# fircarpediem/LSS2_Multimodal_nu

Measured on AMD Instinct MI355X. Metric: BEV frames/sec (6-cam 352x128 -> 200x200x64), full hot path: CamEncode lift + splat + BevEncode, higher is better.
Workload: dtype bf16; 1 GPU; BASELINE configs[1]: model_BEV_TXT LSS hot path, batch=4/GPU, 6 cams 352x128, D=41, 200x200x64 BEV -> BevEncode -> 200x200x4, trunk (EfficientNet) not included: features are the input; batch_per_gpu=4, global_batch=4, parallelism=dp1 (sample-sharded, no collective), precision=bf16

## Files before the change

### lss2_multimodal_nu_amd/csrc/conv_ks.hip

```cpp
#include <stdlib.h>

#include <type_traits>

#include "lss_common.h"

namespace {

constexpr int KS_ROWS = 7;
constexpr int KS_POSB = 64;
constexpr int KS_LDS_MAX = 160 * 1024;

__device__ __attribute__((aligned(128))) unsigned char lss_ks_zero_page[128];

__device__ __forceinline__ void ks_glds16(const void* gsrc, void* lds_wave_base) {
  __builtin_amdgcn_global_load_lds((const __attribute__((address_space(1))) void*)gsrc,
                                   (__attribute__((address_space(3))) void*)lds_wave_base, 16, 0, 0);
}

template <int NCH, class Map>
__device__ __forceinline__ void ks_fill_patch(unsigned char* smem, const unsigned short* ximg, int Cin, int H, int W,
                                              int rows, int pitch, int nposp, int wave, int lane, Map map) {
  const int ppc = nposp >> 4;
  const int q64 = 64 / pitch, r64 = 64 - q64 * pitch;
  const int h = wave & 1;
  const int pos0 = 32 * (wave >> 1) + (lane >> 1);
  int pr = pos0 / pitch, pc = pos0 - pr * pitch;
  const unsigned char* zsrc = lss_ks_zero_page + (lane & 7) * 16;
  const unsigned short* xb = ximg + (2 * h + (lane & 1)) * 8;
  for (int i = wave; i < ppc; i += 4) {
    int iy, ix;
    map(pr, pc, iy, ix);
    const bool in = pr < rows && iy >= 0 && iy < H && ix >= 0 && ix < W;
    const unsigned short* src = xb + (in ? (iy * W + ix) * Cin : 0);
#pragma unroll
    for (int c = 0; c < NCH; ++c)
      ks_glds16(in ? (const void*)(src + c * 32) : (const void*)zsrc,
                smem + ((size_t)(c * 2 + h) * nposp + 32 * (i >> 1)) * 32);
    pr += q64; pc += r64;
    if (pc >= pitch) { pc -= pitch; ++pr; }
  }
}

struct KsStamps {
  unsigned long long* base;
  int tid;
  unsigned long long clk_main = 0;
  __device__ __forceinline__ void stamp(int k) const {
    if (base != nullptr && tid == 0) base[(size_t)blockIdx.x * 8 + k] = __builtin_amdgcn_s_memrealtime();
  }
  __device__ __forceinline__ void main_begin() {
    if (base != nullptr) clk_main = __builtin_amdgcn_s_memtime();
  }
  __device__ __forceinline__ void main_end(const f32x4& first, const f32x4& last) const {
    if (base != nullptr) asm volatile("s_nop 0" ::"v"(first), "v"(last));
    stamp(3);
    if (base != nullptr && tid == 0) base[(size_t)blockIdx.x * 8 + 7] = __builtin_amdgcn_s_memtime() - clk_main;
  }
  __device__ __forceinline__ void drain() const {
    if (base != nullptr) {
      stamp(5);
      asm volatile("s_waitcnt vmcnt(0)" ::: "memory");
      stamp(6);
    }
  }
};

__device__ __forceinline__ void ks_load_affine(const float* scale, const float* shift, int ch, float (&sc)[8], float (&sh)[8]) {
  f32x4 s0 = {1.f, 1.f, 1.f, 1.f}, s1 = s0, h0 = {0.f, 0.f, 0.f, 0.f}, h1 = h0;
  if (scale) { s0 = *reinterpret_cast<const f32x4*>(scale + ch); s1 = *reinterpret_cast<const f32x4*>(scale + ch + 4); }
  if (shift) { h0 = *reinterpret_cast<const f32x4*>(shift + ch); h1 = *reinterpret_cast<const f32x4*>(shift + ch + 4); }
#pragma unroll
  for (int i = 0; i < 4; ++i) { sc[i] = s0[i]; sc[4 + i] = s1[i]; sh[i] = h0[i]; sh[4 + i] = h1[i]; }
}

typedef __attribute__((ext_vector_type(4))) unsigned int u32x4;
__device__ __forceinline__ u32x4 ks_pack8(const float (&v)[8]) {
  return (u32x4){lss_pack_bf2(v[0], v[1]), lss_pack_bf2(v[2], v[3]), lss_pack_bf2(v[4], v[5]), lss_pack_bf2(v[6], v[7])};
}

__device__ __forceinline__ int ks_slot_tile(int slot, int kp, int pxt) {
  const int t = slot + kp;
  return t >= pxt ? t - pxt : t;
}

template <int PXT>
__device__ __forceinline__ void ks_slot_offsets(int (&ab)[PXT], int kp, int pl0, int x_first, int npx, int W,
                                                int rowpitch, int laneoff) {
  const int plast = npx - 1;
  const int yl = (x_first + plast) / W, xl = x_first + plast - yl * W;
  const int y0 = (x_first + pl0) / W, x0 = x_first + pl0 - y0 * W;
  int t = ks_slot_tile(0, kp, PXT);
  int pl = pl0 + t * 16;
  int y = (x_first + pl) / W, x = x_first + pl - y * W;
#pragma unroll
  for (int i = 0; i < PXT; ++i) {
    const bool live = pl < npx;
    ab[i] = ((live ? y : yl) * rowpitch + (live ? x : xl)) * 32 + laneoff;
    pl += 16; x += 16;
    if (x >= W) { x -= W; ++y; }
    if (++t == PXT) { t = 0; pl = pl0; x = x0; y = y0; }
  }
}

template <int NKW, int POS>
__device__ __forceinline__ f32x4 ks_sum_parts(const f32x4& own, const f32x4 (&g)[NKW - 1]) {
  f32x4 sum = POS == 0 ? own : g[0];
#pragma unroll
  for (int q = 1; q < NKW; ++q) {
    const f32x4 pv = q == POS ? own : g[q > POS ? q - 1 : q];
#pragma unroll
    for (int i = 0; i < 4; ++i) sum[i] += pv[i];
  }
  return sum;
}

template <int NKW>
__device__ __forceinline__ f32x4 ks_sum_lds(const f32x4* p0, int kstride) {
  f32x4 sum = p0[0];
#pragma unroll
  for (int k = 1; k < NKW; ++k) {
    const f32x4 pv = p0[k * kstride];
#pragma unroll
    for (int i = 0; i < 4; ++i) sum[i] += pv[i];
  }
  return sum;
}

template <int NKW, class F>
__device__ __forceinline__ void ks_for_pos(int kp, F&& f) {
  if constexpr (NKW == 2) f(std::integral_constant<int, 0>{});
  else if (kp < 2) f(std::integral_constant<int, 0>{});
  else if (kp == 2) f(std::integral_constant<int, 2>{});
  else f(std::integral_constant<int, 3>{});
}

template <bool RES>
__device__ __forceinline__ u32x4 ks_finish8(float (&v)[8], const float (&sc)[8], const float (&sh)[8], const uint4& rv,
                                            bool relu, bool split0) {
  const unsigned int ru[4] = {rv.x, rv.y, rv.z, rv.w};
#pragma unroll
  for (int i = 0; i < 8; ++i) {
    float r;
    if (split0 && i == 0) {
#pragma clang fp contract(off)
      const float p = v[i] * sc[i];
      r = p + sh[i];
    } else {
      r = __builtin_fmaf(v[i], sc[i], sh[i]);
    }
    if constexpr (RES) r += lss_bf2f((unsigned short)((i & 1) ? ru[i >> 1] >> 16 : ru[i >> 1] & 0xffff));
    v[i] = relu ? fmaxf(r, 0.f) : r;
  }
  return ks_pack8(v);
}

struct KsArgs {
  const unsigned short* x;
  const unsigned char* w;
  const float* scale;
  const float* shift;
  const unsigned short* residual;
  unsigned short* y;
  int B, H, W, Cin, Cout, relu, wt;
  int PB;
  int npb;
  int nposp;
  int ncb;
  unsigned long long* stamps;
};

template <int KSW, int NKW, int PXT>
__global__ __launch_bounds__(256, 1) void conv_ks_kernel(const KsArgs a) {
  static_assert(KSW % 9 == 0 && (NKW == 4 || NKW == 2), "a wave's K part is whole chunks of nine taps");
  static_assert(PXT >= NKW - 1, "ks_slot_tile: slot + kp < 2 PXT");
  constexpr int NPW = 4 / NKW;
  constexpr int CPW = KSW / 9;
  constexpr int NT = PXT * NPW;
  extern __shared__ __attribute__((aligned(1024))) unsigned char smem[];
  const int tid = threadIdx.x, lane = tid & 63;
  const int wave = __builtin_amdgcn_readfirstlane(tid >> 6);
  const int kp = wave % NKW, ph = wave / NKW;
  const int n = lane & 15, kq = lane >> 4;
  KsStamps st = {a.stamps, tid};
  st.stamp(0);

  const int t = lss_xcd_order(blockIdx.x, gridDim.x);
  const int cb = t % a.ncb;
  const int pbg = t / a.ncb;
  const int b = pbg / a.npb, pb = pbg - b * a.npb;
  const int HW = a.H * a.W, WP = a.W + 2;
  const int p0 = pb * a.PB;
  const int y_first = p0 / a.W;

  ks_fill_patch<NKW * KSW / 9>(smem, a.x + (size_t)b * HW * a.Cin, a.Cin, a.H, a.W, KS_ROWS, WP, a.nposp, wave, lane,
                               [&](int pr, int pc, int& iy, int& ix) { iy = y_first - 1 + pr; ix = pc - 1; });

#ifdef KS_WPRE_ALL
  constexpr int WPRE = KSW;
#else
  constexpr int WPRE = KSW >= 18 ? 8 : 5;
#endif
  bf16x8 wf[KSW][2];
  const unsigned char* wp = a.w + ((size_t)(cb * NKW + kp) * KSW * 2) * 1024 + lane * 16;
  auto load_w = [&](int s) {
#pragma unroll
    for (int ct = 0; ct < 2; ++ct) wf[s][ct] = *reinterpret_cast<const bf16x8*>(wp + (s * 2 + ct) * 1024);
  };
#pragma unroll
  for (int s = 0; s < WPRE; ++s) load_w(s);

  const int npx = min(a.PB, HW - p0);
  int ab[PXT];
  ks_slot_offsets<PXT>(ab, kp, ph * PXT * 16 + n, p0 - y_first * a.W, npx, a.W, WP,
                       (kq >> 1) * a.nposp * 32 + (kq & 1) * 16);
  st.stamp(1);
  constexpr int NOWN = (PXT + NKW - 1) / NKW;
  const int ch = cb * 32 + kq * 8;
  uint4 rres[NOWN];
#pragma unroll
  for (int k = 0; k < NOWN; ++k) {
    const int j = kp + k * NKW;
    const int pl = (ph * PXT + j) * 16 + n;
    rres[k] = make_uint4(0, 0, 0, 0);
    if (a.residual != nullptr && j < PXT && pl < npx)
      rres[k] = *reinterpret_cast<const uint4*>(a.residual + ((size_t)b * HW + p0 + pl) * a.Cout + ch);
  }
  float sc[8], sh[8];
  ks_load_affine(a.scale, a.shift, ch, sc, sh);
  f32x4 acc[PXT][2];
#pragma unroll
  for (int j = 0; j < PXT; ++j) {
    acc[j][0] = (f32x4){0.f, 0.f, 0.f, 0.f};
    acc[j][1] = (f32x4){0.f, 0.f, 0.f, 0.f};
  }
  asm volatile("s_waitcnt vmcnt(0)" ::: "memory");
  __syncthreads();
  st.stamp(2);

  bf16x8 fb[2][PXT];
  auto load_frags = [&](int buf, int s) {
    const unsigned char* cbase = smem + (size_t)(kp * CPW + s / 9) * a.nposp * KS_POSB;
    const int tap = s % 9;
    const int toff = ((tap / 3) * WP + (tap % 3)) * 32;
#pragma unroll
    for (int j = 0; j < PXT; ++j) fb[buf][j] = *reinterpret_cast<const bf16x8*>(cbase + ab[j] + toff);
  };
  st.main_begin();
  load_frags(0, 0);
#pragma unroll
  for (int s = 0; s < KSW; ++s) {
    if (s + WPRE < KSW) load_w(s + WPRE);
#ifndef KS_DIAG_NOREAD
    if (s + 1 < KSW) load_frags((s + 1) & 1, s + 1);
#endif
    __builtin_amdgcn_sched_barrier(0);
#pragma unroll
    for (int j = 0; j < PXT; ++j) {
#ifdef KS_DIAG_NOMFMA
      asm volatile("" :: "v"(fb[s & 1][j]), "v"(wf[s][0]), "v"(wf[s][1]));
#else
      acc[j][0] = __builtin_amdgcn_mfma_f32_16x16x32_bf16(wf[s][0], fb[s & 1][j], acc[j][0], 0, 0, 0);
      acc[j][1] = __builtin_amdgcn_mfma_f32_16x16x32_bf16(wf[s][1], fb[s & 1][j], acc[j][1], 0, 0, 0);
#endif
    }
    __builtin_amdgcn_sched_barrier(0);
  }

  st.main_end(acc[0][0], acc[PXT - 1][1]);
  __syncthreads();
  f32x4* part = reinterpret_cast<f32x4*>(smem);
#pragma unroll
  for (int i = 0; i < PXT; ++i) {
    if (i % NKW == 0 && kp + i < PXT) continue;
    const int tile = ph * PXT + ks_slot_tile(i, kp, PXT);
#pragma unroll
    for (int ct = 0; ct < 2; ++ct) part[((kp * NT + tile) * 2 + ct) * 64 + lane] = acc[i][ct];
  }
  __syncthreads();
  st.stamp(4);
  const __amdgpu_buffer_rsrc_t yrsrc = __builtin_amdgcn_make_buffer_rsrc(
      a.y, 0, a.wt ? (int)((size_t)a.B * HW * a.Cout * 2) : 0, 0x00020000);
  f32x4 fp[NOWN][2][NKW - 1];
#pragma unroll
  for (int k = 0; k < NOWN; ++k) {
    const int tile = ph * PXT + min(kp + k * NKW, PXT - 1);
#pragma unroll
    for (int ct = 0; ct < 2; ++ct)
#pragma unroll
      for (int m = 0; m < NKW - 1; ++m)
        fp[k][ct][m] = part[(((m < kp ? m : m + 1) * NT + tile) * 2 + ct) * 64 + lane];
  }
  __builtin_amdgcn_sched_barrier(0);
  f32x4 sum[NOWN][2];
  ks_for_pos<NKW>(kp, [&](auto pos) __attribute__((always_inline)) {
#pragma unroll
    for (int k = 0; k < NOWN; ++k)
#pragma unroll
      for (int ct = 0; ct < 2; ++ct) sum[k][ct] = ks_sum_parts<NKW, decltype(pos)::value>(acc[k * NKW][ct], fp[k][ct]);
  });
#pragma unroll
  for (int k = 0; k < NOWN; ++k) {
    const int j = kp + k * NKW;
    const int pl = (ph * PXT + j) * 16 + n;
    const bool live = j < PXT && pl < npx;
    const size_t o = ((size_t)b * HW + p0 + (live ? pl : 0)) * a.Cout + ch;
    float v[8];
#pragma unroll
    for (int ct = 0; ct < 2; ++ct)
#pragma unroll
      for (int i = 0; i < 4; ++i) v[4 * ct + i] = sum[k][ct][i];
    const u32x4 ov = ks_finish8<true>(v, sc, sh, rres[k], a.relu != 0, false);
    if (live) {
      if (a.wt) __builtin_amdgcn_raw_buffer_store_b128(ov, yrsrc, (int)(o * 2), 0, 16);
      else *reinterpret_cast<u32x4*>(a.y + o) = ov;
    }
  }
  st.drain();
}

__global__ void pack_weights_ks_kernel(const float* __restrict__ w, int Cout, int Cin, unsigned short* __restrict__ out,
                                       int dgrad) {
  const size_t ntot = (size_t)Cout * Cin * 9;
  for (size_t e = (size_t)blockIdx.x * 256 + threadIdx.x; e < ntot; e += (size_t)gridDim.x * 256) {
    const int j = e & 7;
    size_t r = e >> 3;
    const int l = r & 63; r >>= 6;
    const int ct = r & 1; r >>= 1;
    const int nks = (Cin >> 5) * 9;
    const int S = r % nks;
    const int cb = r / nks;
    const int m = l & 15, kq = l >> 4;
    const int co = cb * 32 + 8 * (m >> 2) + 4 * ct + (m & 3);
    const int ci = (S / 9) * 32 + kq * 8 + j;
    out[e] = lss_f2bf(dgrad ? w[((size_t)ci * Cout + co) * 9 + (8 - S % 9)] : w[((size_t)co * Cin + ci) * 9 + (S % 9)]);
  }
}

bool ks_enabled() {
  const char* e = getenv("LSS_CONV_KS");
  return e == nullptr || atoi(e) != 0;
}

unsigned long long* ks_stamps_from_env() {
  const char* e = getenv("LSS_KS_STAMPS");
  return e ? reinterpret_cast<unsigned long long*>(strtoull(e, nullptr, 16)) : nullptr;
}

int ks_pack_grid(size_t n) { return (int)((n + 255) / 256 > 4096 ? 4096 : (n + 255) / 256); }

template <class... P>
bool ks_aligned16(const P*... p) {
  return ((reinterpret_cast<uintptr_t>(p) | ...) & 15) == 0;
}

template <auto K, class Args>
int ks_launch(int grid, int lds, const Args& a, hipStream_t st) {
  static bool attr_set[64] = {};
  int dev = -1;
  if (hipGetDevice(&dev) != hipSuccess || dev < 0 || dev >= 64) dev = -1;
  if (dev < 0 || !attr_set[dev]) {
    hipError_t e = hipFuncSetAttribute(reinterpret_cast<const void*>(K), hipFuncAttributeMaxDynamicSharedMemorySize,
                                       KS_LDS_MAX);
    if (e != hipSuccess) return (int)e;
    if (dev >= 0) attr_set[dev] = true;
  }
  hipLaunchKernelGGL(K, dim3(grid), dim3(256), lds, st, a);
  return lss_launch_status();
}

struct KsPlan {
  int ok, lds, grid, variant;
  KsArgs a;
};

KsPlan ks_plan(int B, int H, int W, int Cin, int Cout) {
  KsPlan pl = {};
  KsArgs& p = pl.a;
  if (B <= 0 || H <= 0 || W < 4 || Cout <= 0 || Cout % 32 != 0) return pl;
  if (Cin == 256) { pl.variant = 0; p.PB = 80; }
  else if (Cin == 128) { pl.variant = 1; p.PB = 160; }
  else if (Cin == 64) { pl.variant = 2; p.PB = 320; }
  else return pl;
  p.B = B; p.H = H; p.W = W; p.Cin = Cin; p.Cout = Cout;
  const long long HW = (long long)H * W;
  if (p.PB > 4 * W + 1) return pl;
  p.npb = (int)((HW + p.PB - 1) / p.PB);
  p.ncb = Cout / 32;
  p.nposp = (KS_ROWS * (W + 2) + 31) / 32 * 32;
  const int patch = (Cin / 32) * p.nposp * KS_POSB;
  if (patch > 112 * 1024) return pl;
  const int ntile = p.PB / 16;
  const int red = (pl.variant == 2 ? 2 : 4) * ntile * 2 * 1024;
  pl.lds = patch > red ? patch : red;
  if (pl.lds > KS_LDS_MAX) return pl;
  const long long grid = (long long)B * p.npb * p.ncb;
  if (grid < 64 || grid > 512) return pl;
  if ((long long)B * HW * (Cin > Cout ? Cin : Cout) >= (1LL << 30)) return pl;
  pl.grid = (int)grid;
  pl.ok = 1;
  return pl;
}

struct KsS2Args {
  const unsigned short* x;
  const unsigned char* w;
  const float* scale;
  const float* shift;
  unsigned short* y;
  unsigned short* y2;
  int B, H, W, Cin, Cout, relu;
  int Ho, Wo, pitch;
  int PB, npb, nposp, ncb;
  unsigned long long* stamps;
};

constexpr int KS2_PXT = 3;
constexpr int KS2_CT = 4;

template <int NKW>
__global__ __launch_bounds__(256, 1) void conv_ks_s2_dual_kernel(const KsS2Args a) {
  static_assert(NKW == 4 || NKW == 2, "one 32-channel chunk of nine taps per K part");
  constexpr int NPW = 4 / NKW, PXT = KS2_PXT, CT = KS2_CT, NT = PXT * NPW, NCH = NKW;
  constexpr bool OWN = NKW == 2;
  extern __shared__ __attribute__((aligned(1024))) unsigned char smem[];
  const int tid = threadIdx.x, lane = tid & 63;
  const int wave = __builtin_amdgcn_readfirstlane(tid >> 6);
  const int kp = wave % NKW, ph = wave / NKW;
  const int n = lane & 15, kq = lane >> 4;
  KsStamps st = {a.stamps, tid};
  st.stamp(0);

  const int t = lss_xcd_order(blockIdx.x, gridDim.x);
  const int cb = t % a.ncb;
  const int pbg = t / a.ncb;
  const int b = pbg / a.npb, pb = pbg - b * a.npb;
  const int HWo = a.Ho * a.Wo, WP = a.pitch;
  const int p0 = pb * a.PB;
  const int r0 = p0 / a.Wo;

  ks_fill_patch<NCH>(smem, a.x + (size_t)b * a.H * a.W * a.Cin, a.Cin, a.H, a.W, KS_ROWS, WP, a.nposp, wave, lane,
                     [&](int pr, int pc, int& iy, int& ix) {
                       iy = 2 * r0 - 1 + pr; ix = pc < a.Wo ? 2 * pc : 2 * (pc - a.Wo) - 1;
                     });

  constexpr int WPRE = 4;
  bf16x8 wf[9][CT], wd[CT];
  const unsigned char* wp = a.w + ((size_t)(cb * NKW + kp) * 10 * CT) * 1024 + lane * 16;
  auto load_w = [&](int s) {
#pragma unroll
    for (int ct = 0; ct < CT; ++ct) wf[s][ct] = *reinterpret_cast<const bf16x8*>(wp + (s * CT + ct) * 1024);
  };
#pragma unroll
  for (int s = 0; s < WPRE; ++s) load_w(s);
#pragma unroll
  for (int ct = 0; ct < CT; ++ct) wd[ct] = *reinterpret_cast<const bf16x8*>(wp + (9 * CT + ct) * 1024);

  const int npx = min(a.PB, HWo - p0);
  const int rot = OWN ? kp : 0;
  int ab[PXT];
  ks_slot_offsets<PXT>(ab, rot, ph * PXT * 16 + n, p0 - r0 * a.Wo, npx, a.Wo, 2 * WP,
                       (kq >> 1) * a.nposp * 32 + (kq & 1) * 16);
  st.stamp(1);
  f32x4 acc[PXT][CT], acc2[PXT][CT];
#pragma unroll
  for (int j = 0; j < PXT; ++j)
#pragma unroll
    for (int ct = 0; ct < CT; ++ct) {
      acc[j][ct] = (f32x4){0.f, 0.f, 0.f, 0.f};
      acc2[j][ct] = (f32x4){0.f, 0.f, 0.f, 0.f};
    }
  asm volatile("s_waitcnt vmcnt(0)" ::: "memory");
  __syncthreads();
  st.stamp(2);

  bf16x8 fb[2][PXT];
  auto load_frags = [&](int buf, int s) {
    const unsigned char* cbase = smem + (size_t)kp * a.nposp * KS_POSB;
    const int ky = s / 3, kx = s % 3;
    const int toff = (ky * WP + (kx == 1 ? 0 : kx == 0 ? a.Wo : a.Wo + 1)) * 32;
#pragma unroll
    for (int j = 0; j < PXT; ++j) fb[buf][j] = *reinterpret_cast<const bf16x8*>(cbase + ab[j] + toff);
  };
  st.main_begin();
  load_frags(0, 0);
#pragma unroll
  for (int s = 0; s < 9; ++s) {
    if (s + WPRE < 9) load_w(s + WPRE);
    if (s + 1 < 9) load_frags((s + 1) & 1, s + 1);
    __builtin_amdgcn_sched_barrier(0);
#pragma unroll
    for (int j = 0; j < PXT; ++j)
#pragma unroll
      for (int ct = 0; ct < CT; ++ct)
        acc[j][ct] = __builtin_amdgcn_mfma_f32_16x16x32_bf16(wf[s][ct], fb[s & 1][j], acc[j][ct], 0, 0, 0);
    if (s == 4) {
#pragma unroll
      for (int j = 0; j < PXT; ++j)
#pragma unroll
        for (int ct = 0; ct < CT; ++ct)
          acc2[j][ct] = __builtin_amdgcn_mfma_f32_16x16x32_bf16(wd[ct], fb[0][j], acc2[j][ct], 0, 0, 0);
    }
    __builtin_amdgcn_sched_barrier(0);
  }

  st.main_end(acc[0][0], acc[PXT - 1][CT - 1]);
  __syncthreads();
  f32x4* part = reinterpret_cast<f32x4*>(smem);
#pragma unroll
  for (int i = 0; i < PXT; ++i) {
    if (OWN && i % NKW == 0 && kp + i < PXT) continue;
    const int tile = ph * PXT + ks_slot_tile(i, rot, PXT);
#pragma unroll
    for (int ct = 0; ct < CT; ++ct) {
      part[(((0 * NKW + kp) * NT + tile) * CT + ct) * 64 + lane] = acc[i][ct];
      part[(((1 * NKW + kp) * NT + tile) * CT + ct) * 64 + lane] = acc2[i][ct];
    }
  }
  float sc[2][2][8], sh[2][2][8];
#pragma unroll
  for (int o = 0; o < 2; ++o)
#pragma unroll
    for (int g = 0; g < 2; ++g)
      ks_load_affine(a.scale, a.shift, o * a.Cout + cb * 64 + g * 32 + kq * 8, sc[o][g], sh[o][g]);
  __syncthreads();
  st.stamp(4);
  constexpr int NOWN = (PXT + NKW - 1) / NKW;
  if constexpr (!OWN) {
#pragma unroll
    for (int k = 0; k < NOWN; ++k) {
      const int j = kp + k * NKW;
      if (j >= PXT) break;
      const int tile = ph * PXT + j;
      const int pl = tile * 16 + n;
      const bool live = pl < npx;
      const size_t opix = ((size_t)b * HWo + p0 + (live ? pl : 0)) * a.Cout + cb * 64 + kq * 8;
#pragma unroll
      for (int o = 0; o < 2; ++o)
#pragma unroll
        for (int g = 0; g < 2; ++g) {
          float v[8];
#pragma unroll
          for (int tt = 0; tt < 2; ++tt) {
            const f32x4 sum = ks_sum_lds<NKW>(part + ((o * NKW * NT + tile) * CT + 2 * g + tt) * 64 + lane, NT * CT * 64);
#pragma unroll
            for (int i = 0; i < 4; ++i) v[4 * tt + i] = sum[i];
          }
#pragma unroll
          for (int i = 0; i < 8; ++i) {
            v[i] = v[i] * sc[o][g][i] + sh[o][g][i];
            if (o == 0 && a.relu) v[i] = fmaxf(v[i], 0.f);
          }
          if (live) *reinterpret_cast<u32x4*>((o == 0 ? a.y : a.y2) + opix + g * 32) = ks_pack8(v);
        }
    }
    st.drain();
    return;
  }
  f32x4 fp[NOWN][2][CT][NKW - 1];
#pragma unroll
  for (int k = 0; k < NOWN; ++k) {
    const int tile = ph * PXT + min(kp + k * NKW, PXT - 1);
#pragma unroll
    for (int o = 0; o < 2; ++o)
#pragma unroll
      for (int ct = 0; ct < CT; ++ct)
#pragma unroll
        for (int m = 0; m < NKW - 1; ++m)
          fp[k][o][ct][m] = part[(((o * NKW + (m < kp ? m : m + 1)) * NT + tile) * CT + ct) * 64 + lane];
  }
  __builtin_amdgcn_sched_barrier(0);
  f32x4 sum[NOWN][2][CT];
  ks_for_pos<NKW>(kp, [&](auto pos) __attribute__((always_inline)) {
#pragma unroll
    for (int k = 0; k < NOWN; ++k)
#pragma unroll
      for (int ct = 0; ct < CT; ++ct) {
        sum[k][0][ct] = ks_sum_parts<NKW, decltype(pos)::value>(acc[k * NKW][ct], fp[k][0][ct]);
        sum[k][1][ct] = ks_sum_parts<NKW, decltype(pos)::value>(acc2[k * NKW][ct], fp[k][1][ct]);
      }
  });
#pragma unroll
  for (int k = 0; k < NOWN; ++k) {
    const int j = kp + k * NKW;
    const int pl = (ph * PXT + j) * 16 + n;
    const bool live = j < PXT && pl < npx;
    const size_t opix = ((size_t)b * HWo + p0 + (live ? pl : 0)) * a.Cout + cb * 64 + kq * 8;
#pragma unroll
    for (int o = 0; o < 2; ++o)
#pragma unroll
      for (int g = 0; g < 2; ++g) {
        float v[8];
#pragma unroll
        for (int tt = 0; tt < 2; ++tt)
#pragma unroll
          for (int i = 0; i < 4; ++i) v[4 * tt + i] = sum[k][o][2 * g + tt][i];
        const u32x4 ov = ks_finish8<false>(v, sc[o][g], sh[o][g], make_uint4(0, 0, 0, 0), o == 0 && a.relu, o == 0);
        if (live) *reinterpret_cast<u32x4*>((o == 0 ? a.y : a.y2) + opix + g * 32) = ov;
      }
  }
  st.drain();
}

__global__ void pack_weights_ks_s2_dual_kernel(const float* __restrict__ w1, const float* __restrict__ wd, int Cout,
                                               int Cin, unsigned short* __restrict__ out) {
  const size_t ntot = (size_t)Cout * Cin * 10;
  const int nch = Cin >> 5;
  for (size_t e = (size_t)blockIdx.x * 256 + threadIdx.x; e < ntot; e += (size_t)gridDim.x * 256) {
    const int j = e & 7;
    size_t r = e >> 3;
    const int l = r & 63; r >>= 6;
    const int ct = r & 3; r >>= 2;
    const int s = r % 10; r /= 10;
    const int kp = r % nch;
    const int cb = r / nch;
    const int m = l & 15, kq = l >> 4;
    const int co = cb * 64 + 32 * (ct >> 1) + 8 * (m >> 2) + 4 * (ct & 1) + (m & 3);
    const int ci = kp * 32 + kq * 8 + j;
    out[e] = lss_f2bf(s < 9 ? w1[((size_t)co * Cin + ci) * 9 + s] : wd[(size_t)co * Cin + ci]);
  }
}

struct KsS2Plan {
  int ok, lds, grid, nkw;
  KsS2Args a;
};

KsS2Plan ks_s2_plan(int B, int H, int W, int Cin, int Cout) {
  KsS2Plan pl = {};
  KsS2Args& p = pl.a;
  if (B <= 0 || H < 2 || W < 4 || Cout <= 0 || Cout % 64 != 0) return pl;
  if (Cin == 128) pl.nkw = 4;
  else if (Cin == 64) pl.nkw = 2;
  else return pl;
  p.B = B; p.H = H; p.W = W; p.Cin = Cin; p.Cout = Cout;
  p.Ho = (H - 1) / 2 + 1; p.Wo = (W - 1) / 2 + 1;
  p.pitch = 2 * p.Wo + 1;
  p.PB = 16 * KS2_PXT * (4 / pl.nkw);
  if (p.PB > 2 * p.Wo + 1) return pl;
  const long long HWo = (long long)p.Ho * p.Wo;
  p.npb = (int)((HWo + p.PB - 1) / p.PB);
  p.ncb = Cout / 64;
  p.nposp = (KS_ROWS * p.pitch + 31) / 32 * 32;
  const int patch = (Cin / 32) * p.nposp * KS_POSB;
  if (patch > 112 * 1024) return pl;
  const int red = 2 * pl.nkw * (p.PB / 16) * KS2_CT * 1024;
  pl.lds = patch > red ? patch : red;
  if (pl.lds > KS_LDS_MAX) return pl;
  const long long grid = (long long)B * p.npb * p.ncb;
  if (grid < 64 || grid > 512) return pl;
  if ((long long)B * H * W * Cin >= (1LL << 30) || (long long)B * HWo * Cout >= (1LL << 30)) return pl;
  pl.grid = (int)grid;
  pl.ok = 1;
  return pl;
}

constexpr int ST_TH = 12, ST_TW = 16;
constexpr int ST_PR = 2 * ST_TH + 5, ST_PW = 2 * ST_TW + 5;
constexpr int ST_NE = ST_TW + 3;
constexpr int ST_NPOSP = (ST_PR * ST_PW + 31) / 32 * 32;
constexpr int ST_LDS = 2 * ST_NPOSP * KS_POSB;
constexpr int ST_KS = 98;
constexpr int ST_WPRE = 8;
constexpr int ST_PXT = ST_TH / 2;

struct KsStemArgs {
  const unsigned short* x;
  const unsigned char* w;
  const float* scale;
  const float* shift;
  unsigned short* y;
  int B, H, W, Cout, relu;
  int Ho, Wo, nty, ntx, ncb;
  unsigned long long* stamps;
};

__global__ __launch_bounds__(256, 1) void conv_ks_stem_kernel(const KsStemArgs a) {
  constexpr int PXT = ST_PXT, Cin = 64;
  extern __shared__ __attribute__((aligned(1024))) unsigned char smem[];
  const int tid = threadIdx.x, lane = tid & 63;
  const int wave = __builtin_amdgcn_readfirstlane(tid >> 6);
  const int g = wave & 1, ph = wave >> 1;
  const int n = lane & 15, kq = lane >> 4;
  KsStamps st = {a.stamps, tid};
  st.stamp(0);

  const int t = lss_xcd_order(blockIdx.x, gridDim.x);
  const int cb = t % a.ncb;
  const int tg = t / a.ncb;
  const int npi = a.nty * a.ntx;
  const int b = tg / npi, ti = tg - b * npi;
  const int ty = ti / a.ntx, tx = ti - ty * a.ntx;
  const int oy0 = ty * ST_TH, ox0 = tx * ST_TW;
  const int iy0 = 2 * oy0 - 3, ix0 = 2 * ox0 - 3;

  ks_fill_patch<2>(smem, a.x + (size_t)b * a.H * a.W * Cin, Cin, a.H, a.W, ST_PR, ST_PW, ST_NPOSP, wave, lane,
                   [&](int pr, int pc, int& iy, int& ix) {
                     iy = iy0 + pr; ix = ix0 + (pc < ST_NE ? 2 * pc : 2 * (pc - ST_NE) + 1);
                   });

  bf16x8 wf[ST_KS][2];
  const unsigned char* wp = a.w + ((size_t)cb * ST_KS * 4 + 2 * g) * 1024 + lane * 16;
  auto load_w = [&](int s) {
#pragma unroll
    for (int ct = 0; ct < 2; ++ct) wf[s][ct] = *reinterpret_cast<const bf16x8*>(wp + (s * 4 + ct) * 1024);
  };
#pragma unroll
  for (int s = 0; s < ST_WPRE; ++s) load_w(s);

  const int ab0 = (2 * (ph * PXT) * ST_PW + n) * 32 + (kq >> 1) * ST_NPOSP * 32 + (kq & 1) * 16;
  st.stamp(1);
  f32x4 acc[PXT][2];
#pragma unroll
  for (int j = 0; j < PXT; ++j) {
    acc[j][0] = (f32x4){0.f, 0.f, 0.f, 0.f};
    acc[j][1] = (f32x4){0.f, 0.f, 0.f, 0.f};
  }
  const int ch = cb * 64 + g * 32 + kq * 8;
  float sc[8], sh[8];
  ks_load_affine(a.scale, a.shift, ch, sc, sh);
  asm volatile("s_waitcnt vmcnt(0)" ::: "memory");
  __syncthreads();
  st.stamp(2);

  bf16x8 fb[2][PXT];
  auto load_frags = [&](int buf, int s) {
    const int tap = s >> 1, ky = tap / 7, kx = tap % 7;
    const int toff = (ky * ST_PW + ((kx & 1) ? ST_NE + (kx >> 1) : (kx >> 1))) * 32;
    const unsigned char* cbase = smem + (size_t)(s & 1) * 2 * ST_NPOSP * 32 + ab0 + toff;
#pragma unroll
    for (int j = 0; j < PXT; ++j) fb[buf][j] = *reinterpret_cast<const bf16x8*>(cbase + j * (2 * ST_PW * 32));
  };
  st.main_begin();
  load_frags(0, 0);
#pragma unroll
  for (int s = 0; s < ST_KS; ++s) {
    if (s + ST_WPRE < ST_KS) load_w(s + ST_WPRE);
    if (s + 1 < ST_KS) load_frags((s + 1) & 1, s + 1);
    __builtin_amdgcn_sched_barrier(0);
#pragma unroll
    for (int j = 0; j < PXT; ++j) {
      acc[j][0] = __builtin_amdgcn_mfma_f32_16x16x32_bf16(wf[s][0], fb[s & 1][j], acc[j][0], 0, 0, 0);
      acc[j][1] = __builtin_amdgcn_mfma_f32_16x16x32_bf16(wf[s][1], fb[s & 1][j], acc[j][1], 0, 0, 0);
    }
    __builtin_amdgcn_sched_barrier(0);
  }
  st.main_end(acc[0][0], acc[PXT - 1][1]);
  st.stamp(4);

  const int ox = ox0 + n;
#pragma unroll
  for (int j = 0; j < PXT; ++j) {
    const int oy = oy0 + ph * PXT + j;
    float v[8];
#pragma unroll
    for (int i = 0; i < 4; ++i) { v[i] = acc[j][0][i]; v[4 + i] = acc[j][1][i]; }
#pragma unroll
    for (int i = 0; i < 8; ++i) {
      v[i] = v[i] * sc[i] + sh[i];
      if (a.relu) v[i] = fmaxf(v[i], 0.f);
    }
    if (oy < a.Ho && ox < a.Wo)
      *reinterpret_cast<u32x4*>(a.y + (((size_t)b * a.Ho + oy) * a.Wo + ox) * a.Cout + ch) = ks_pack8(v);
  }
  st.drain();
}

__global__ void pack_weights_ks_stem_kernel(const float* __restrict__ w, int Cout, unsigned short* __restrict__ out) {
  const size_t ntot = (size_t)Cout * 64 * 49;
  for (size_t e = (size_t)blockIdx.x * 256 + threadIdx.x; e < ntot; e += (size_t)gridDim.x * 256) {
    const int j = e & 7;
    size_t r = e >> 3;
    const int l = r & 63; r >>= 6;
    const int ct = r & 3; r >>= 2;
    const int S = r % ST_KS;
    const int cb = r / ST_KS;
    const int m = l & 15, kq = l >> 4;
    const int co = cb * 64 + 32 * (ct >> 1) + 8 * (m >> 2) + 4 * (ct & 1) + (m & 3);
    const int ci = (S & 1) * 32 + kq * 8 + j;
    out[e] = lss_f2bf(w[((size_t)co * 64 + ci) * 49 + (S >> 1)]);
  }
}

struct KsStemPlan {
  int ok, grid;
  KsStemArgs a;
};

KsStemPlan ks_stem_plan(int B, int H, int W, int Cin, int Cout) {
  KsStemPlan pl = {};
  KsStemArgs& p = pl.a;
  if (B <= 0 || H <= 0 || W <= 0 || Cin != 64 || Cout <= 0 || Cout % 64 != 0) return pl;
  p.B = B; p.H = H; p.W = W; p.Cout = Cout;
  p.Ho = (H - 1) / 2 + 1; p.Wo = (W - 1) / 2 + 1;
  if (p.Ho < ST_TH || p.Wo < ST_TW) return pl;
  p.nty = (p.Ho + ST_TH - 1) / ST_TH; p.ntx = (p.Wo + ST_TW - 1) / ST_TW;
  p.ncb = Cout / 64;
  const long long grid = (long long)B * p.nty * p.ntx * p.ncb;
  if (grid < 32 || grid > 256) return pl;
  if ((long long)B * H * W * Cin >= (1LL << 30) || (long long)B * p.Ho * p.Wo * Cout >= (1LL << 30)) return pl;
  pl.grid = (int)grid;
  pl.ok = 1;
  return pl;
}

}

extern "C" int lss_conv2d_ks_ok(int B, int H, int W, int Cin, int Cout) {
  return ks_enabled() && ks_plan(B, H, W, Cin, Cout).ok;
}

extern "C" size_t lss_conv2d_ks_packed_weight_bytes(int Cout, int Cin) {
  if (Cout <= 0 || Cout % 32 != 0 || (Cin != 64 && Cin != 128 && Cin != 256)) return 0;
  return (size_t)Cout * Cin * 9 * 2;
}

extern "C" int lss_conv2d_pack_weights_ks(const float* w_oihw, int Cout, int Cin, void* w_packed, void* stream) {
  LSS_CHECK_PTR(w_oihw); LSS_CHECK_PTR(w_packed);
  if (lss_conv2d_ks_packed_weight_bytes(Cout, Cin) == 0) return LSS_E_SHAPE;
  hipLaunchKernelGGL(pack_weights_ks_kernel, dim3(ks_pack_grid((size_t)Cout * Cin * 9)), dim3(256), 0, lss_stream(stream), w_oihw, Cout, Cin,
                     reinterpret_cast<unsigned short*>(w_packed), 0);
  return lss_launch_status();
}

extern "C" int lss_conv2d_pack_weights_ks_dgrad(const float* w_oihw, int Cout, int Cin, void* w_packed, void* stream) {
  LSS_CHECK_PTR(w_oihw); LSS_CHECK_PTR(w_packed);
  if (lss_conv2d_ks_packed_weight_bytes(Cin, Cout) == 0) return LSS_E_SHAPE;
  hipLaunchKernelGGL(pack_weights_ks_kernel, dim3(ks_pack_grid((size_t)Cout * Cin * 9)), dim3(256), 0, lss_stream(stream), w_oihw, Cin, Cout,
                     reinterpret_cast<unsigned short*>(w_packed), 1);
  return lss_launch_status();
}

int lss_conv_ks_launch(const void* x, const void* w_ks, const float* scale, const float* shift, const void* residual,
                       void* y, int B, int H, int W, int Cin, int Cout, int relu, int wt, hipStream_t st) {
  KsPlan p = ks_plan(B, H, W, Cin, Cout);
  if (!p.ok) return LSS_E_SHAPE;
  if (relu != 0 && relu != 1) return LSS_E_LAYOUT;
  if (!ks_aligned16(x, y, w_ks, residual)) return LSS_E_ALIGN;
  KsArgs& a = p.a;
  a.x = reinterpret_cast<const unsigned short*>(x);
  a.w = reinterpret_cast<const unsigned char*>(w_ks);
  a.scale = scale; a.shift = shift;
  a.residual = reinterpret_cast<const unsigned short*>(residual);
  a.y = reinterpret_cast<unsigned short*>(y);
  a.relu = relu; a.wt = wt;
  a.stamps = ks_stamps_from_env();
  if (p.variant == 0) return ks_launch<conv_ks_kernel<18, 4, 5>>(p.grid, p.lds, a, st);
  if (p.variant == 1) return ks_launch<conv_ks_kernel<9, 4, 10>>(p.grid, p.lds, a, st);
  return ks_launch<conv_ks_kernel<9, 2, 10>>(p.grid, p.lds, a, st);
}

extern "C" int lss_conv2d_ks_s2_dual_ok(int B, int H, int W, int Cin, int Cout) {
  return ks_enabled() && ks_s2_plan(B, H, W, Cin, Cout).ok;
}

extern "C" size_t lss_conv2d_ks_s2_dual_packed_weight_bytes(int Cout, int Cin) {
  if (Cout <= 0 || Cout % 64 != 0 || (Cin != 64 && Cin != 128)) return 0;
  return (size_t)Cout * Cin * 10 * 2;
}

extern "C" int lss_conv2d_pack_weights_ks_s2_dual(const float* w1_oihw, const float* wd_oi, int Cout, int Cin,
                                                  void* w_packed, void* stream) {
  LSS_CHECK_PTR(w1_oihw); LSS_CHECK_PTR(wd_oi); LSS_CHECK_PTR(w_packed);
  if (lss_conv2d_ks_s2_dual_packed_weight_bytes(Cout, Cin) == 0) return LSS_E_SHAPE;
  hipLaunchKernelGGL(pack_weights_ks_s2_dual_kernel, dim3(ks_pack_grid((size_t)Cout * Cin * 10)), dim3(256), 0, lss_stream(stream), w1_oihw, wd_oi, Cout,
                     Cin, reinterpret_cast<unsigned short*>(w_packed));
  return lss_launch_status();
}

extern "C" int lss_conv2d_ks_s2_dual_fwd(const void* x, const void* w_packed, const float* scale, const float* shift,
                                         void* y, void* y2, int B, int H, int W, int Cin, int Cout, int relu,
                                         void* stream) {
  LSS_CHECK_PTR(x); LSS_CHECK_PTR(w_packed); LSS_CHECK_PTR(y); LSS_CHECK_PTR(y2);
  KsS2Plan p = ks_s2_plan(B, H, W, Cin, Cout);
  if (!p.ok) return LSS_E_SHAPE;
  if (relu != 0 && relu != 1) return LSS_E_LAYOUT;
  if (!ks_aligned16(x, y, y2, w_packed, scale, shift)) return LSS_E_ALIGN;
  KsS2Args& a = p.a;
  a.x = reinterpret_cast<const unsigned short*>(x);
  a.w = reinterpret_cast<const unsigned char*>(w_packed);
  a.scale = scale; a.shift = shift;
  a.y = reinterpret_cast<unsigned short*>(y);
  a.y2 = reinterpret_cast<unsigned short*>(y2);
  a.relu = relu;
  a.stamps = ks_stamps_from_env();
  return p.nkw == 4 ? ks_launch<conv_ks_s2_dual_kernel<4>>(p.grid, p.lds, a, lss_stream(stream))
                    : ks_launch<conv_ks_s2_dual_kernel<2>>(p.grid, p.lds, a, lss_stream(stream));
}

extern "C" int lss_conv2d_ks_stem_ok(int B, int H, int W, int Cin, int Cout) {
  return ks_enabled() && ks_stem_plan(B, H, W, Cin, Cout).ok;
}

extern "C" size_t lss_conv2d_ks_stem_packed_weight_bytes(int Cout, int Cin) {
  if (Cout <= 0 || Cout % 64 != 0 || Cin != 64) return 0;
  return (size_t)Cout * Cin * 49 * 2;
}

extern "C" int lss_conv2d_pack_weights_ks_stem(const float* w_oihw, int Cout, int Cin, void* w_packed, void* stream) {
  LSS_CHECK_PTR(w_oihw); LSS_CHECK_PTR(w_packed);
  if (lss_conv2d_ks_stem_packed_weight_bytes(Cout, Cin) == 0) return LSS_E_SHAPE;
  hipLaunchKernelGGL(pack_weights_ks_stem_kernel, dim3(ks_pack_grid((size_t)Cout * Cin * 49)), dim3(256), 0, lss_stream(stream), w_oihw, Cout,
                     reinterpret_cast<unsigned short*>(w_packed));
  return lss_launch_status();
}

extern "C" int lss_conv2d_ks_stem_fwd(const void* x, const void* w_packed, const float* scale, const float* shift,
                                      void* y, int B, int H, int W, int Cin, int Cout, int relu, void* stream) {
  LSS_CHECK_PTR(x); LSS_CHECK_PTR(w_packed); LSS_CHECK_PTR(y);
  KsStemPlan p = ks_stem_plan(B, H, W, Cin, Cout);
  if (!p.ok) return LSS_E_SHAPE;
  if (relu != 0 && relu != 1) return LSS_E_LAYOUT;
  if (!ks_aligned16(x, y, w_packed, scale, shift)) return LSS_E_ALIGN;
  KsStemArgs& a = p.a;
  a.x = reinterpret_cast<const unsigned short*>(x);
  a.w = reinterpret_cast<const unsigned char*>(w_packed);
  a.scale = scale; a.shift = shift;
  a.y = reinterpret_cast<unsigned short*>(y);
  a.relu = relu;
  a.stamps = ks_stamps_from_env();
  return ks_launch<conv_ks_stem_kernel>(p.grid, ST_LDS, a, lss_stream(stream));
}
```

Measured before the change: 12150 frames/s.

## Add 64-channel-per-block conv variant sharing one patch and trim patch rows loaded

Adds a variant of the implicit-GEMM 3x3 conv in which each block computes two 32-channel output groups: the wave pairs split channels rather than pixels, and the pixel block shrinks to 160. One LDS input patch is then reused across 64 output channels. The patch fill also computes how many image rows the pixel range actually touches and loads only those, skipping unused rows. This trades grid size and per-block pixel parallelism for less repeated patch loading, and it changes the LDS sizing; it is enabled by default through an environment flag.

```diff
diff --git a/lss2_multimodal_nu_amd/csrc/conv_ks.hip b/lss2_multimodal_nu_amd/csrc/conv_ks.hip
--- a/lss2_multimodal_nu_amd/csrc/conv_ks.hip
+++ b/lss2_multimodal_nu_amd/csrc/conv_ks.hip
@@ -7,6 +7,7 @@
 namespace {
 
 constexpr int KS_ROWS = 7;
+constexpr int KS_ROWS_CH64 = 5;
 constexpr int KS_POSB = 64;
 constexpr int KS_LDS_MAX = 160 * 1024;
 
@@ -20,7 +21,7 @@
 template <int NCH, class Map>
 __device__ __forceinline__ void ks_fill_patch(unsigned char* smem, const unsigned short* ximg, int Cin, int H, int W,
                                               int rows, int pitch, int nposp, int wave, int lane, Map map) {
-  const int ppc = nposp >> 4;
+  const int ppc = min(nposp >> 4, (rows * pitch + 31) >> 5 << 1);
   const int q64 = 64 / pitch, r64 = 64 - q64 * pitch;
   const int h = wave & 1;
   const int pos0 = 32 * (wave >> 1) + (lane >> 1);
@@ -39,6 +40,19 @@
     pr += q64; pc += r64;
     if (pc >= pitch) { pc -= pitch; ++pr; }
   }
+}
+
+template <int SPAN>
+__device__ __forceinline__ int ks_rows_read(int x_first, int npx, int W) {
+#ifdef KS_DIAG_FILL7
+  return KS_ROWS;
+#else
+  const int e = x_first + npx - 1;
+  int yl = 0;
+#pragma unroll
+  for (int k = 1; k < SPAN; ++k) yl += e >= k * W;
+  return yl + 3;
+#endif
 }
 
 struct KsStamps {
@@ -169,13 +183,13 @@
   unsigned long long* stamps;
 };
 
-template <int KSW, int NKW, int PXT>
+template <int KSW, int NKW, int PXT, bool CH2 = false>
 __global__ __launch_bounds__(256, 1) void conv_ks_kernel(const KsArgs a) {
   static_assert(KSW % 9 == 0 && (NKW == 4 || NKW == 2), "a wave's K part is whole chunks of nine taps");
   static_assert(PXT >= NKW - 1, "ks_slot_tile: slot + kp < 2 PXT");
-  constexpr int NPW = 4 / NKW;
+  static_assert(!CH2 || NKW == 2, "two channel parts x two K parts");
   constexpr int CPW = KSW / 9;
-  constexpr int NT = PXT * NPW;
+  constexpr int NT = PXT * (4 / NKW);
   extern __shared__ __attribute__((aligned(1024))) unsigned char smem[];
   const int tid = threadIdx.x, lane = tid & 63;
   const int wave = __builtin_amdgcn_readfirstlane(tid >> 6);
@@ -185,14 +199,18 @@
   st.stamp(0);
 
   const int t = lss_xcd_order(blockIdx.x, gridDim.x);
-  const int cb = t % a.ncb;
+  const int cb = CH2 ? 2 * (t % a.ncb) + ph : t % a.ncb;
+  const int pp = CH2 ? 0 : ph;
   const int pbg = t / a.ncb;
   const int b = pbg / a.npb, pb = pbg - b * a.npb;
   const int HW = a.H * a.W, WP = a.W + 2;
   const int p0 = pb * a.PB;
   const int y_first = p0 / a.W;
 
-  ks_fill_patch<NKW * KSW / 9>(smem, a.x + (size_t)b * HW * a.Cin, a.Cin, a.H, a.W, KS_ROWS, WP, a.nposp, wave, lane,
+  const int npx = min(a.PB, HW - p0);
+
+  ks_fill_patch<NKW * KSW / 9>(smem, a.x + (size_t)b * HW * a.Cin, a.Cin, a.H, a.W,
+                               ks_rows_read<CH2 ? 3 : 5>(p0 - y_first * a.W, npx, a.W), WP, a.nposp, wave, lane,
                                [&](int pr, int pc, int& iy, int& ix) { iy = y_first - 1 + pr; ix = pc - 1; });
 
 #ifdef KS_WPRE_ALL
@@ -209,9 +227,8 @@
 #pragma unroll
   for (int s = 0; s < WPRE; ++s) load_w(s);
 
-  const int npx = min(a.PB, HW - p0);
   int ab[PXT];
-  ks_slot_offsets<PXT>(ab, kp, ph * PXT * 16 + n, p0 - y_first * a.W, npx, a.W, WP,
+  ks_slot_offsets<PXT>(ab, kp, pp * PXT * 16 + n, p0 - y_first * a.W, npx, a.W, WP,
                        (kq >> 1) * a.nposp * 32 + (kq & 1) * 16);
   st.stamp(1);
   constexpr int NOWN = (PXT + NKW - 1) / NKW;
@@ -220,7 +237,7 @@
 #pragma unroll
   for (int k = 0; k < NOWN; ++k) {
     const int j = kp + k * NKW;
-    const int pl = (ph * PXT + j) * 16 + n;
+    const int pl = (pp * PXT + j) * 16 + n;
     rres[k] = make_uint4(0, 0, 0, 0);
     if (a.residual != nullptr && j < PXT && pl < npx)
       rres[k] = *reinterpret_cast<const uint4*>(a.residual + ((size_t)b * HW + p0 + pl) * a.Cout + ch);
@@ -301,7 +318,7 @@
 #pragma unroll
   for (int k = 0; k < NOWN; ++k) {
     const int j = kp + k * NKW;
-    const int pl = (ph * PXT + j) * 16 + n;
+    const int pl = (pp * PXT + j) * 16 + n;
     const bool live = j < PXT && pl < npx;
     const size_t o = ((size_t)b * HW + p0 + (live ? pl : 0)) * a.Cout + ch;
     float v[8];
@@ -338,6 +355,11 @@
 
 bool ks_enabled() {
   const char* e = getenv("LSS_CONV_KS");
+  return e == nullptr || atoi(e) != 0;
+}
+
+bool ks_ch64_enabled() {
+  const char* e = getenv("LSS_KS_CH64");
   return e == nullptr || atoi(e) != 0;
 }
 
@@ -398,6 +420,16 @@
   if ((long long)B * HW * (Cin > Cout ? Cin : Cout) >= (1LL << 30)) return pl;
   pl.grid = (int)grid;
   pl.ok = 1;
+  if (pl.variant == 2 && Cout % 64 == 0 && ks_ch64_enabled()) {
+    pl.variant = 3;
+    p.PB = 160;
+    p.npb = (int)((HW + p.PB - 1) / p.PB);
+    p.ncb = Cout / 64;
+    p.nposp = (KS_ROWS_CH64 * (W + 2) + 31) / 32 * 32;
+    const int patch64 = (Cin / 32) * p.nposp * KS_POSB;
+    pl.lds = patch64 > red ? patch64 : red;
+    pl.grid = B * p.npb * p.ncb;
+  }
   return pl;
 }
 
@@ -437,6 +469,7 @@
   const int HWo = a.Ho * a.Wo, WP = a.pitch;
   const int p0 = pb * a.PB;
   const int r0 = p0 / a.Wo;
+  const int npx = min(a.PB, HWo - p0);
 
   ks_fill_patch<NCH>(smem, a.x + (size_t)b * a.H * a.W * a.Cin, a.Cin, a.H, a.W, KS_ROWS, WP, a.nposp, wave, lane,
                      [&](int pr, int pc, int& iy, int& ix) {
@@ -455,7 +488,6 @@
 #pragma unroll
   for (int ct = 0; ct < CT; ++ct) wd[ct] = *reinterpret_cast<const bf16x8*>(wp + (9 * CT + ct) * 1024);
 
-  const int npx = min(a.PB, HWo - p0);
   const int rot = OWN ? kp : 0;
   int ab[PXT];
   ks_slot_offsets<PXT>(ab, rot, ph * PXT * 16 + n, p0 - r0 * a.Wo, npx, a.Wo, 2 * WP,
@@ -846,6 +878,7 @@
   a.stamps = ks_stamps_from_env();
   if (p.variant == 0) return ks_launch<conv_ks_kernel<18, 4, 5>>(p.grid, p.lds, a, st);
   if (p.variant == 1) return ks_launch<conv_ks_kernel<9, 4, 10>>(p.grid, p.lds, a, st);
+  if (p.variant == 3) return ks_launch<conv_ks_kernel<9, 2, 10, true>>(p.grid, p.lds, a, st);
   return ks_launch<conv_ks_kernel<9, 2, 10>>(p.grid, p.lds, a, st);
 }
 
```

Measured after the change: 12220 frames/s (median of 6 runs). About the same (+0.6%).
